# tpatten/squirrel_motion_planner

Hardware: AMD Instinct MI355X
Metric: collision-checked samples/sec + time-to-first-feasible-path, 8-DoF, 5 cm octomap (higher is better)
Workload: dtype f64

## Files before the change

squirrel_motion_planner_amd/csrc/smp_kernels.hip:

```cpp
#include <hip/hip_runtime.h>

#include <vector>

#include "smp_collide.h"
#include "smp_math.h"
#include "smp_plan.h"
#include "smp_types.h"

extern "C" __device__ __attribute__((const)) unsigned long long __ockl_wfred_min_u64(unsigned long long);
extern "C" __device__ __attribute__((const)) unsigned long long __ockl_wfred_max_u64(unsigned long long);

namespace smp {

constexpr int CHECK_CT = 32;

__shared__ RobotDev g_rb;
__shared__ MapCfg g_mc;
__shared__ WideStash g_wk;

__device__ __forceinline__ void stage_model(const RobotDev* rb, const MapCfg* mc, RobotDev* rbl, MapCfg* mcl) {
  static_assert(sizeof(RobotDev) % 8 == 0 && sizeof(MapCfg) % 4 == 0, "staging granularity");
  for (int i = threadIdx.x; i < (int)(sizeof(RobotDev) / 8); i += BLOCK)
    reinterpret_cast<uint64_t*>(rbl)[i] = reinterpret_cast<const uint64_t*>(rb)[i];
  for (int i = threadIdx.x; i < (int)(sizeof(MapCfg) / 4); i += BLOCK)
// ... 335 lines not shown
  NodeRef sel;
  double sel_start[NJ], sel_target[NJ];
  double csp[3], best_nv;
  double sol[3];
  double wd[BLOCK / 64];
  unsigned long long wk[BLOCK / 64];
  int wi[BLOCK / 64];
  long long wcount[BLOCK / 64];
  ScoutRec sr;
  PreRec prer;
  int prer_ok;
#ifdef SMP_TRACE
  int trole;
  unsigned tn;
  long long tit;
#endif
  int sp_on, sp_stage, sp_go[2];
  double fnn_d;
  int fnn_id;
#ifdef SMP_SCAN_PROF
  unsigned long long spc_t;
#endif
  int sc_same[MAX_SCOUTS];
  unsigned sc_seen, sc_dead;
  int asked[SCOUT_SLOTS];
  int asked_conn[SCOUT_SLOTS];
  int asked_pre[SCOUT_SLOTS];
  int conn_rec;
  int two_scouts;
  unsigned sc_mod;
  unsigned rw_at0;
  int n_at0;
  int sc_t, sc_rerun;
  int rb_go[2];
  long long sc_k;
  int eg_hit[MAXE];
  int eg_rec[MAXE];
  int rec_grp;
  int rec_all, ev_job;
  double pc_q[2][PATCH_K][NJ];
};

__shared__ PlanLds g_L;

struct Ctx {
  SceneDev sc;
  QueryDev Q;
};

#ifdef SMP_TRACE
#ifndef SMP_TRACE_IT0
#define SMP_TRACE_IT0 3000
#endif
#ifndef SMP_TRACE_IT1
#define SMP_TRACE_IT1 3040
#endif
constexpr unsigned TLOG_CAP = 1u << 18, TLOG_ROLE = TLOG_CAP / 4;
__device__ unsigned long long g_tlog[TLOG_CAP];
__device__ unsigned g_tlog_n[4];
#define TR()                                                                                                  \
  if (threadIdx.x == 0 && g_L.tit >= SMP_TRACE_IT0 && g_L.tit < SMP_TRACE_IT1 && g_L.tn < TLOG_ROLE) {        \
    g_tlog[g_L.trole * TLOG_ROLE + g_L.tn] =                                                                   \
        ((unsigned long long)g_L.trole << 62) | ((unsigned long long)((g_L.tit - SMP_TRACE_IT0) & 0xff) << 54) | \
        ((unsigned long long)(__LINE__ & 0x3fff) << 40) | (wall_clock64() & 0xffffffffffull);                  \
    g_tlog_n[g_L.trole] = ++g_L.tn;                                                                            \
  }
// ... 1687 lines not shown
      const int c = threadIdx.x / NJ, j = threadIdx.x - c * NJ;
      const int sl = base + c, k = sl / J.np1, i = sl - k * J.np1;
      J.tq[c][j] = J.start[k][j] + i * J.step[k][j];
    }
    if (threadIdx.x < TILE_CT_MAX) J.T.coll[threadIdx.x] = 0;
    __syncthreads();
  }
  const TileOrder order{J.tgrp, J.tord, J.first, false};
  collide_wide((&g_rb), K, ct, nc, J.tq, self, map, J.T, sk ? &order : nullptr, prof);
  unsigned m = 0;
  for (int c = 0; c < nc; ++c) m |= (J.T.coll[c] ? 1u : 0u) << c;
  if (sync_after) __syncthreads();
  return m;
}

__device__ __noinline__ unsigned job_tile_mask_out(const Ctx& C, JobLds& J, int t, int seq) {
  const WideConst K = wide_const_load(g_wk, C.sc);
  return job_tile_mask(C, K, J, t, nullptr, seq);
}

enum { OV_NONE = 0, OV_NEAR_EXPAND = 1, OV_NN = 2, OV_NEAR_XN = 3 };
__device__ void overlap_work(const Ctx& C, int ov, int t);
__device__ __forceinline__ bool take_spec(int ov) {
  const bool hit = uni(g_L.spec) == ov;
  __syncthreads();
  if (hit && threadIdx.x == 0) {
    (ov == OV_NN ? g_L.S.nn_nodes : g_L.S.near_nodes) += g_L.spec_cnt;
    g_L.spec = OV_NONE;
  }
  __syncthreads();
  return hit;
}

__device__ __forceinline__ void edge_validity_job(const Ctx& C, int E, int pslot, int ov, int ovt, bool sfv) {
  JobBoard* jb = C.Q.jb;
  auto& J = g_L.u.job;
  const int np1 = g_L.S.n_pts + 1;
  const int W = max(1, C.Q.nworkers);
  if (threadIdx.x < 64) {
    const int e = threadIdx.x;
    const bool need = e < E && g_L.eg_need[e] && g_L.eg_hit[e] < 0;
    const unsigned long long m = __ballot(need);
    const int k = __popcll(m & ((1ull << e) - 1));
    if (need) J.emap[k] = e;
    if (e == 0) {
      const int ne = __popcll(m);
      J.E = ne;
      J.np1 = np1;
      J.nslots = ne * np1;
      J.ct = job_tile_ct(ne * np1, W, C.Q.tile_ct);
      J.ntiles = (ne * np1 + J.ct - 1) / J.ct;
      J.self = g_L.S.self; J.map = g_L.S.map;
      J.seq = ++g_L.job_seq;
#ifdef SMP_NO_SKIP
      J.skip = 0;
#else
      J.skip = J.ntiles > W;
#endif
      J.sfv = J.skip && sfv;
    }
  }
  if (threadIdx.x < E) g_L.eg_first[threadIdx.x] = np1;
  __syncthreads();
  const int ne = uni(J.E), nt = uni(J.ntiles), seq = uni(J.seq), ct = uni(J.ct);
  if (ne == 0) {
    overlap_work(C, OV_NONE, ovt);
    return;
  }
  const unsigned long long tj0 = threadIdx.x == 0 ? wall_clock64() : 0;
  for (int it = threadIdx.x; it < ne * NJ; it += BLOCK) {
    const int k = it / NJ, j = it - k * NJ, e = J.emap[k];
    J.start[k][j] = g_L.eg_start[e][j];
    J.step[k][j] = g_L.eg_step[e][j];
  }
  for (int t = threadIdx.x; t < nt; t += BLOCK) J.rdone[t] = 0;
  if (threadIdx.x < ne) J.first[threadIdx.x] = np1;
  __syncthreads();
  for (int i = threadIdx.x; i < 1 + 32 * ne; i += BLOCK) {
    unsigned w;
    if (i == 0) {
      w = (unsigned)ne | (unsigned)np1 << 8 | (unsigned)(J.self != 0) << 16 | (unsigned)(J.map != 0) << 17 |
          (unsigned)J.skip << 19 | (unsigned)J.sfv << 20 | (unsigned)__builtin_ctz((unsigned)J.ct) << 21;
    } else {
      const int m = i - 1, k = m >> 5, r = m & 31, j = (r & 15) >> 1;
      const unsigned long long bits = (unsigned long long)__double_as_longlong(r < 16 ? J.start[k][j] : J.step[k][j]);
      w = (r & 1) ? (unsigned)(bits >> 32) : (unsigned)bits;
    }
    st_agent(&jb->pay[i], granule(seq, w));
  }
#ifdef SMP_JOB_PROF
  if (threadIdx.x == 0) st_agent(&jb->dbg[0], wall_clock64());
#endif
  PROF_BEGIN();
  if (threadIdx.x == 0) { g_L.S.prof[P_TFK] += _pt - tj0; g_L.S.prof[P_TTEST]++; }
  TR();
  if (threadIdx.x == 0) g_L.in_job = 1;
  __syncthreads();
  overlap_work(C, ov, ovt);
  if (threadIdx.x == 0) g_L.in_job = 0;
  TR();
  const bool skip = uni(J.skip) != 0;
  for (int t = W - 1; t < nt; t += W) {
    const unsigned m = job_tile_mask_out(C, J, t, skip ? seq : -1);
    if (threadIdx.x == 0) {
      J.rmask[t] = m;
      J.rdone[t] = 1;
      if (skip) st_agent(&jb->res[t], granule(seq, m));
    }
  }
  __syncthreads();
  const unsigned long long tj1 = threadIdx.x == 0 ? wall_clock64() : 0;
  if (threadIdx.x == 0) g_L.S.prof[P_TCHAIN] += tj1 - _pt;
  unsigned long long t_prog = tj1, t_wait = tj1;
  int last_left = 1 << 30;
  for (int k = 0;; k ^= 1) {
    if (threadIdx.x < 64) {
      int left = 0;
      for (int t = threadIdx.x; t < nt; t += 64) {
        if (J.rdone[t]) continue;
        const unsigned long long v = ld_agent(&jb->res[t]);
        if ((int)(v >> 32) == seq) { J.rmask[t] = (unsigned)v; J.rdone[t] = 1; }
        else ++left;
      }
      left = __ockl_wfred_add_i32(left);
      if (threadIdx.x == 0) {
        const unsigned long long now = wall_clock64();
        if (left != last_left) { last_left = left; t_prog = now; }
        int st = left == 0 ? 1 : (now - t_prog > 800ull ? 2 : 0);
        if (st != 1 && now - t_wait > 200000000ull) {
          g_L.S.status = -5;
          g_L.S.phase = 2;
          g_L.S.prof[28] = (unsigned long long)left;
          g_L.S.prof[29] = (unsigned long long)nt;
          g_L.S.prof[31] = (unsigned long long)seq;
          st = 1;
        }
        J.go[k] = st;
      }
    }
    __syncthreads();
    const int go = uni(J.go[k]);
    if (go == 1) break;
    if (go == 2) {
      if (threadIdx.x < 64) {
        int cand = 1 << 30;
        for (int t = threadIdx.x; t < nt; t += 64)
          if (!J.rdone[t]) { cand = t; break; }
        cand = __ockl_wfred_min_i32(cand);
        if (threadIdx.x == 0) J.steal = cand < nt ? cand : -1;
      }
      __syncthreads();
      const int t = uni(J.steal);
      if (t >= 0) {
        const unsigned m = job_tile_mask_out(C, J, t, -1);
        if (threadIdx.x == 0) { J.rmask[t] = m; J.rdone[t] = 1; }
      }
// ... 773 lines not shown
      }
    }
    if (e < MAXE) g_L.eg_rec[e] = m;
    const unsigned long long miss = __ballot(e < E && m < 0);
    if (e == 0) { g_L.rec_grp = sgrp; g_L.rec_all = miss == 0; }
  }
  __syncthreads();
  return uni(g_L.rec_all) != 0;
}

__device__ void edge_costs_rec(int E) {
  const int np = g_L.S.n_pts;
  if (threadIdx.x < E * NJ) {
    const int e = threadIdx.x / NJ, j = threadIdx.x - e * NJ;
    const double st = (g_L.eg_target[e][j] - g_L.eg_start[e][j]) / double(np);
    g_L.eg_step[e][j] = st;
    g_L.eg_end[e][j] = g_L.eg_start[e][j] + np * st;
  } else if (threadIdx.x >= 256 && threadIdx.x < 256 + E * 3) {
    const int i = threadIdx.x - 256, e = i / 3, k = i - e * 3;
    const double a = g_L.sr.e[g_L.eg_rec[e]].acc[k];
    g_L.eg_acc[e][k] = a;
    g_L.eg_cost[e][k] = g_L.eg_base[e][k] + a;
  }
  __syncthreads();
}

__device__ __noinline__ void local_tile(const Ctx& C, int nc) {
  const TileOrder order{g_L.tile_e, g_L.tile_i, g_L.eg_first, false};
  collide_tile<PLAN_CT>((&g_rb), C.sc, (&g_mc), nc, g_L.u.tile.tq, g_L.S.self, g_L.S.map, g_L.u.tile.T, &order,
                        &g_L.S.prof[P_TFK]);
}

__device__ __forceinline__ void edge_validity(const Ctx& C, int E, bool stop_first_valid, int pslot, int ov = 0, int ovt = 0,
                              int sgrp = -1) {
  const int np1 = g_L.S.n_pts + 1;
  if (threadIdx.x == 0) g_L.count_slot = pslot + 4;
  TR();
  if (C.Q.jb) {
    const bool matched = uni(g_L.rec_grp) == sgrp && sgrp >= 0;
    const bool rec = sgrp >= 0 && (matched || spec_stage(C, sgrp));
    TR();
    if (threadIdx.x < 64) {
      const int e = threadIdx.x;
      const bool need = e < E && g_L.eg_need[e];
      int hit = -2;
      if (rec && need) {
        if (matched) {
          const int k = g_L.eg_rec[e];
          if (k >= 0 && g_L.sr.e[k].first >= 0) hit = g_L.sr.e[k].first;
        } else {
          const int g0 = sgrp == SC_EXPAND ? 0 : sgrp == SC_CHOOSE ? SCOUT_CHOOSE0 : SCOUT_REWIRE0;
          const int gn = sgrp == SC_EXPAND ? 1 : sgrp == SC_CHOOSE ? g_L.sr.n_choose : g_L.sr.n_rewire;
          const int d = e < gn ? e : -1;
          for (int u = 0; u < gn; ++u) {
            const int k = g0 + (d < 0 ? u : (u == 0 ? d : (u <= d ? u - 1 : u)));
            const ScoutEdge& R = g_L.sr.e[k];
            if (R.first >= 0 && same8(g_L.eg_start[e], R.s) && same8(g_L.eg_target[e], R.g)) { hit = R.first; break; }
          }
        }
      }
      if (e < MAXE) g_L.eg_hit[e] = hit;
      const unsigned long long mh = __ballot(need && hit >= 0), mm = __ballot(need && hit < 0);
      if (rec && e == 0) { g_L.S.sc_edge_hit += __popcll(mh); g_L.S.sc_edge_miss += __popcll(mm); }
      if (mm == 0 && e < E) g_L.eg_first[e] = need ? hit : np1;
      if (e == 0) {
        g_L.ev_job = mm != 0;
        g_L.rec_grp = -1;
        if (mm == 0) g_L.spec = OV_NONE;
      }
    }
    __syncthreads();
    if (!uni(g_L.ev_job)) { TR(); return; }
    edge_validity_job(C, E, pslot, ov, ovt, stop_first_valid);
    if (threadIdx.x < E && g_L.eg_hit[threadIdx.x] >= 0) g_L.eg_first[threadIdx.x] = g_L.eg_hit[threadIdx.x];
    __syncthreads();
    TR();
    return;
  }
  if (threadIdx.x < E) { g_L.eg_first[threadIdx.x] = np1; g_L.eg_ptr[threadIdx.x] = 0; }
  __syncthreads();
  for (;;) {
    if (threadIdx.x < 64) {
      const int e = threadIdx.x;
      const bool live = e < E && g_L.eg_need[e] && g_L.eg_first[e] >= np1;
      const int ptr = e < E ? g_L.eg_ptr[e] : np1;
      bool stop = false;
      if (stop_first_valid) {
        const unsigned long long m = __ballot(live);
        if (m) stop = __shfl(ptr, __builtin_ctzll(m)) >= np1;
      }
      const int rem = (live && ptr < np1) ? np1 - ptr : 0;
      int inc = rem;
      for (int off = 1; off < 32; off <<= 1) {
        int v = __shfl_up(inc, off);
        if (e >= off) inc += v;
      }
      const int start = inc - rem;
      const int take = stop ? 0 : max(0, min(rem, PLAN_CT - start));
      for (int i = 0; i < take; ++i) { g_L.tile_e[start + i] = e; g_L.tile_i[start + i] = ptr + i; }
      if (e < E) g_L.eg_ptr[e] = ptr + take;
      const int total = __shfl(inc, 31);
      if (e == 0) g_L.tile_n = stop ? 0 : min(PLAN_CT, total);
    }
    __syncthreads();
    const int nc = uni(g_L.tile_n);
    if (nc == 0) break;
    if (threadIdx.x < nc * NJ) {
      int c = threadIdx.x / NJ, j = threadIdx.x - c * NJ;
      int e = g_L.tile_e[c];
      g_L.u.tile.tq[c][j] = g_L.eg_start[e][j] + g_L.tile_i[c] * g_L.eg_step[e][j];
    }
    __syncthreads();
// ... 709 lines not shown
    __syncthreads();
    if (C.Q.jb && rec_match(C, E, SC_CHOOSE)) edge_costs_rec(E);
    else edge_costs(C, E);
    if (threadIdx.x < E) g_L.eg_need[threadIdx.x] = g_L.eg_cost[threadIdx.x][0] <= g_L.xn.c[0];
    for (int e = E + threadIdx.x; e < MAXE; e += BLOCK) g_L.eg_need[e] = 0;
    __syncthreads();
    edge_validity(C, E, true, P_XCHOOSE, 0, 0, SC_CHOOSE);
    count_edges(E, true);
    if (threadIdx.x == 0) {
      if (g_L.found >= 0) {
        g_L.ext_bp = 1;
        g_L.n_via = 0;
        g_L.nn_t = g_L.S.n[t];
        load_node(C, t, g_L.eg_near[g_L.found], &g_L.cur);
      }
    }
    __syncthreads();
    if (uni(g_L.found) >= 0) {
      via_chain(C, g_L.xn.q);
      if (threadIdx.x == 0) {
        g_L.xn.id = g_L.sel.id;
        g_L.xn.parent = g_L.sel.parent;
        for (int j = 0; j < NJ; ++j) g_L.xn.q[j] = g_L.sel.q[j];
        for (int k = 0; k < 3; ++k) g_L.xn.c[k] = g_L.sel.c[k];
        for (int j = 0; j < NJ; ++j) { g_L.en_start[j] = g_L.sel_start[j]; g_L.en_target[j] = g_L.sel_target[j]; }
      }
      __syncthreads();
      insert_via(C, t);
    }
  }
  __syncthreads();
}

__device__ void rewire_count(const TreeDev& T) {
  if (threadIdx.x < 64) {
    const int n = g_L.nk, lane = threadIdx.x;
    const int m = n >= g_L.S.max_near ? g_L.S.max_near : n;
    bool ok = false;
    if (lane < m) {
      int hv = g_L.n_hi - 1 - lane;
      BCHK(hv, MAX_NEAR, __LINE__, 9);
      int v = g_L.hi_i[hv];
      BCHK(v, g_L.S.cap, __LINE__, 9);
      ok = g_L.xn.c[0] < T.cost[v];
    }
    const int cnt = __popcll(__ballot(ok));
    if (lane == 0) g_L.cnt = cnt;
  }
  __syncthreads();
}

__device__ void rewire(const Ctx& C, int t) {
  const int cap = g_L.S.cap;
  const TreeDev& T = C.Q.tr[t];
  rewire_count(T);
  const int cnt = uni(g_L.cnt);
  if (cnt == 0) return;
  if (threadIdx.x < cnt) {
    int e = threadIdx.x;
    int pos = g_L.n_hi - 1 - e;
    int v = g_L.hi_i[pos];
    NodeRef nd;
    load_node(C, t, v, &nd);
    for (int j = 0; j < NJ; ++j) { g_L.eg_start[e][j] = g_L.xn.q[j]; g_L.eg_target[e][j] = nd.q[j]; }
    for (int k = 0; k < 3; ++k) g_L.eg_base[e][k] = g_L.xn.c[k];
    g_L.eg_near[e] = v;
  }
// ... 964 lines not shown
  if (threadIdx.x == 0) {
    S.n[t] = Xn;
    S.n[1 - t] = XBn;
    S.prof[26]++;
    R.cn.ok = 0;
    R.pre.ok = 0;
    R.nn.ok = 0; R.ex.ok = 0; R.nr.ok = 0; R.n_choose = 0; R.n_rewire = 0; R.cc.ok = 0; R.cc.nfirst = -1;
  }
  __syncthreads();
  return true;
}

__device__ void scout_iteration(const Ctx& C, long long it, int t, int X, int opt, unsigned ver, int XB) {
  QState& S = g_L.S;
  ScoutRec& R = g_L.sr;
  ScoutBoard* sb = C.Q.scb;
  JobBoard* jb = C.Q.jb;
  const int par = (int)(it & (SCOUT_SLOTS - 1));
  const unsigned tag = (unsigned)(it + 1);
  (void)jb;
  unsigned long long _ts = threadIdx.x == 0 ? pclk() : 0;
#ifdef SMP_TRACE
  if (threadIdx.x == 0) g_L.tit = it;
#endif
  TR();
  if (threadIdx.x == 0) {
    S.prof[30]++;
    S.n[t] = X;
    S.n[1 - t] = XB;
    R.cn.ok = 0;
    R.pre.ok = 0;
    R.nn.ok = 0; R.ex.ok = 0; R.nr.ok = 0; R.n_choose = 0; R.n_rewire = 0; R.cc.ok = 0; R.cc.nfirst = -1;
  }
  if (opt) sc_publish(C, par, tag, SC_STARTED);
  if (threadIdx.x < 64) {
    const JobBoard* lb = C.Q.sampler_jb;
    const unsigned want = ring_tag(it, ver);
    const unsigned long long t0 = wall_clock64();
    int ok = 0;
    for (;;) {
      unsigned long long v = 0;
      if (threadIdx.x < 2 * NJ) v = ld_agent(&lb->ring[it % SMP_RING].g[threadIdx.x]);
      const bool cur = threadIdx.x >= 2 * NJ || (unsigned)(v >> 32) == want;
      if (__ballot(!cur) == 0) {
        const unsigned hi = (unsigned)odd_lane_of_pair((int)(unsigned)v);
        if (threadIdx.x < 2 * NJ && !(threadIdx.x & 1))
          g_L.xr[threadIdx.x >> 1] = __longlong_as_double((long long)(((unsigned long long)hi << 32) | (unsigned)v));
        ok = 1;
        break;
      }
      if (__builtin_amdgcn_readfirstlane((int)(wall_clock64() - t0 > 2000))) break;
      __builtin_amdgcn_s_sleep(2);
    }
    if (threadIdx.x == 0) g_L.flag = ok;
  }
  __syncthreads();
  SC_PHASE(0);
  TR();
  if (!uni(g_L.flag) && !opt) {
    scout_pre_publish(C, par, tag, false);
    return;
  }
  if (!uni(g_L.flag)) {
    sc_copy_out(sb, par, &R.nn, sizeof(ScoutNN));
    sc_copy_out(sb, par, &R.nr, sizeof(ScoutNear));
    sc_copy_out(sb, par, &R.cn, sizeof(ScoutConnect));
    sc_copy_out(sb, par, &R.pre, sizeof(ScoutPre));
    sc_copy_out(sb, par, &R.n_choose, 4 * sizeof(int));
    sc_end(C, par, tag, opt);
    return;
  }
  int rp = 0;
redo:
  if (opt && sc_moved(C)) return;
  int nid;
// ... 7 lines not shown
    for (int j = 0; j < NJ; ++j) { nq[j] = g_L.nn.q[j]; xe[j] = g_L.xr[j]; }
    double s = 0.0;
#pragma unroll
    for (int j = 0; j < NJ; ++j) { const double d = xe[j] - nq[j]; s += d * d; }
    const double d = sqrt(s);
    const double nn_l = g_L.nn.q[lane & 7];
    double x_l = g_L.xr[lane & 7];
    step_towards_w(rev_mask(&g_rb), nq, xe, S.step, lane, nn_l, x_l);
    if (lane < NJ) {
      R.nn.q[lane] = g_L.xr[lane];
      g_L.ext[lane] = x_l;
      g_L.eg_start[0][lane] = nn_l;
      g_L.eg_target[0][lane] = x_l;
    } else if (lane < NJ + 3) {
      const int k = lane - NJ;
      R.nn.c[k] = g_L.nn.c[k];
      g_L.eg_base[0][k] = g_L.nn.c[k];
    } else if (lane == NJ + 3) {
      R.nn.d = d < 10000.0 ? d : 10000.0;
      R.nn.id = nid; R.nn.X = X; R.nn.t = t; R.nn.ok = 1;
      g_L.eg_need[0] = 1;
    }
  }
  __syncthreads();
  if (opt) {
    sc_copy_out(sb, par, &R.nn, sizeof(ScoutNN));
    sc_publish(C, par, tag, SC_NN);
  }
  SC_PHASE(1);
  TR();
  if (opt && sc_moved(C)) return;
  edge_costs(C, 1);
  if (threadIdx.x == 0) {
    for (int j = 0; j < NJ; ++j) { R.ex.ext[j] = g_L.eg_target[0][j]; R.ex.step[j] = g_L.eg_step[0][j]; R.ex.end[j] = g_L.eg_end[0][j]; }
    for (int k = 0; k < 3; ++k) R.ex.acc[k] = g_L.eg_acc[0][k];
    R.ex.ok = 1;
  }
  if (threadIdx.x == 0) g_L.spec = OV_NONE;
  const bool spec_conn = !opt && !sc_stale(C, tag);
  int cid_s = 0;
  if (spec_conn) {
    const int tb = 1 - t;
    [[clang::always_inline]] cid_s = nearest(C, tb, g_L.eg_end[0]);
    if (threadIdx.x == 0) {
      load_node(C, tb, cid_s, &g_L.xc);
      for (int j = 0; j < NJ; ++j) { g_L.eg_start[1][j] = g_L.xc.q[j]; g_L.eg_target[1][j] = g_L.eg_end[0][j]; }
      for (int k = 0; k < 3; ++k) g_L.eg_base[1][k] = g_L.xc.c[k];
      g_L.eg_need[1] = 1;
    }
    for (int e = 2 + threadIdx.x; e < MAXE; e += BLOCK) g_L.eg_need[e] = 0;
    __syncthreads();
    edge_costs(C, 2);
    [[clang::always_inline]] edge_validity(C, 2, false, P_XEXPAND, OV_NONE, t);
  } else {
    [[clang::always_inline]] edge_validity(C, 1, false, P_XEXPAND, opt ? OV_NEAR_EXPAND : OV_NONE, t);
  }
  if (threadIdx.x == 0) {
    for (int j = 0; j < NJ; ++j) { R.e[0].s[j] = g_L.eg_start[0][j]; R.e[0].g[j] = g_L.eg_target[0][j]; }
    for (int k = 0; k < 3; ++k) R.e[0].acc[k] = g_L.eg_acc[0][k];
    R.e[0].first = g_L.eg_first[0];
    const int f = g_L.eg_first[0];
    g_L.ext_nn = f > S.n_pts;
    if (g_L.ext_nn) {
      for (int j = 0; j < NJ; ++j) g_L.xn.q[j] = g_L.eg_end[0][j];
      for (int k = 0; k < 3; ++k) g_L.xn.c[k] = g_L.eg_cost[0][k];
    } else {
      for (int j = 0; j < NJ; ++j) g_L.xn.q[j] = g_L.xr[j];
      g_L.xn.c[0] = 10000.0; g_L.xn.c[1] = 0.0; g_L.xn.c[2] = 0.0;
    }
    g_L.xn.id = X;
    g_L.xn.parent = g_L.nn.id;
    g_L.ext_bp = 0;
  }
  __syncthreads();
  if (!opt && (C.Q.pre_refresh & 1) && rp < 2 && pre_newer(C, t, X, XB)) {
    X = uni(g_L.cnt);
    XB = uni(g_L.found);
    rp++;
    goto redo;
  }
  if (opt) {
    sc_copy_out(sb, par, &R.e[0], sizeof(ScoutEdge));
    sc_copy_out(sb, par, &R.ex, sizeof(ScoutExpand));
  }
  if (spec_conn && uni(g_L.ext_nn)) {
    const int tb = 1 - t;
    const int cid = cid_s;
    if (threadIdx.x < NJ) {
      const int j = threadIdx.x;
      g_L.eg_start[0][j] = g_L.eg_start[1][j]; g_L.eg_target[0][j] = g_L.eg_target[1][j];
      g_L.eg_step[0][j] = g_L.eg_step[1][j]; g_L.eg_end[0][j] = g_L.eg_end[1][j];
    }
    if (threadIdx.x < 3) {
      const int k = threadIdx.x;
      g_L.eg_base[0][k] = g_L.eg_base[1][k]; g_L.eg_acc[0][k] = g_L.eg_acc[1][k]; g_L.eg_cost[0][k] = g_L.eg_cost[1][k];
    }
    if (threadIdx.x == 0) {
      g_L.eg_first[0] = g_L.eg_first[1];
      double s = 0.0;
      for (int j = 0; j < NJ; ++j) { double d = g_L.xn.q[j] - g_L.xc.q[j]; s += d * d; }
      const double d = sqrt(s);
      for (int j = 0; j < NJ; ++j) R.cn.q[j] = g_L.xn.q[j];
      R.cn.d = d < 10000.0 ? d : 10000.0;
      R.cn.id = cid; R.cn.X = XB; R.cn.t = tb;
    }
    __syncthreads();
    if (threadIdx.x == 0) {
      for (int j = 0; j < NJ; ++j) { R.cn.e.s[j] = g_L.eg_start[0][j]; R.cn.e.g[j] = g_L.eg_target[0][j]; }
      for (int k = 0; k < 3; ++k) { R.cn.e.acc[k] = g_L.eg_acc[0][k]; R.cn.c[k] = g_L.xc.c[k]; }
      R.cn.e.first = g_L.eg_first[0];
      R.cn.ok = 1;
    }
    __syncthreads();
    scout_pre_connect(C, par, tb);
  }
  if (!opt && (C.Q.pre_refresh & 2) && rp < 2 && pre_newer(C, t, X, XB)) {
    X = uni(g_L.cnt);
    XB = uni(g_L.found);
    rp++;
    goto redo;
  }
  if (!opt) {
    scout_pre_publish(C, par, tag, true);
    return;
  }
  if (sc_stale(C, tag)) {
    sc_copy_out(sb, par, &R.nr, sizeof(ScoutNear));
    sc_copy_out(sb, par, &R.n_choose, 4 * sizeof(int));
    sc_publish(C, par, tag, SC_DONE);
    return;
  }
  sc_publish(C, par, tag, SC_EXPAND);
  SC_PHASE(2);
  TR();
  if (sc_moved(C)) return;
  if (!(uni(g_L.ext_nn) && take_spec(OV_NEAR_EXPAND))) {
    [[clang::always_inline]] near_set<20>(C, t, g_L.xn.q, X);
  }
  if (threadIdx.x < 20) {
    R.nr.lo_i[threadIdx.x] = g_L.lo_i[threadIdx.x]; R.nr.lo_c[threadIdx.x] = g_L.lo_c[threadIdx.x];
    R.nr.hi_i[threadIdx.x] = g_L.hi_i[threadIdx.x]; R.nr.hi_c[threadIdx.x] = g_L.hi_c[threadIdx.x];
  }
  if (threadIdx.x == 0) {
    for (int j = 0; j < NJ; ++j) R.nr.q[j] = g_L.xn.q[j];
    R.nr.nk = g_L.nk; R.nr.n_lo = g_L.n_lo; R.nr.n_hi = g_L.n_hi;
    R.nr.X = X; R.nr.t = t; R.nr.ok = 1;
  }
  __syncthreads();
  sc_copy_out(sb, par, &R.nr, sizeof(ScoutNear));
  sc_publish(C, par, tag, SC_NEAR);
  SC_PHASE(3);
  TR();
  if (sc_moved(C)) return;
  if (threadIdx.x < 64) {
    const int E = choose_prefix();
    if (threadIdx.x == 0) {
      g_L.cnt = E;
      g_L.found = -1;
    }
  }
  __syncthreads();
  const int E = uni(g_L.cnt);
  if (E > 0) {
    if (threadIdx.x < E) {
      const int e = threadIdx.x;
      NodeRef nd;
      load_node(C, t, g_L.lo_i[e], &nd);
      for (int j = 0; j < NJ; ++j) { g_L.eg_start[e][j] = nd.q[j]; g_L.eg_target[e][j] = g_L.xn.q[j]; }
      for (int k = 0; k < 3; ++k) g_L.eg_base[e][k] = nd.c[k];
      g_L.eg_near[e] = nd.id;
    }
    __syncthreads();
    edge_costs(C, E);
    if (threadIdx.x < E) g_L.eg_need[threadIdx.x] = g_L.eg_cost[threadIdx.x][0] <= g_L.xn.c[0];
    for (int e = E + threadIdx.x; e < MAXE; e += BLOCK) g_L.eg_need[e] = 0;
    __syncthreads();
    [[clang::always_inline]] edge_validity(C, E, false, P_XCHOOSE);
    if (threadIdx.x < E) {
      const int e = threadIdx.x;
      ScoutEdge& w = R.e[SCOUT_CHOOSE0 + e];
      for (int j = 0; j < NJ; ++j) { w.s[j] = g_L.eg_start[e][j]; w.g[j] = g_L.eg_target[e][j]; }
      for (int k = 0; k < 3; ++k) w.acc[k] = g_L.eg_acc[e][k];
      w.first = g_L.eg_need[e] ? g_L.eg_first[e] : -1;
    }
    if (threadIdx.x < 64) {
      const bool fr = (int)threadIdx.x < E && g_L.eg_need[threadIdx.x] && g_L.eg_first[threadIdx.x] > S.n_pts;
      const unsigned long long fm = __ballot(fr);
      if (threadIdx.x == 0) {
        R.n_choose = E;
        if (fm) g_L.found = (int)__builtin_ctzll(fm);
      }
    }
    __syncthreads();
  }
  sc_copy_out(sb, par, &R.n_choose, 4 * sizeof(int));
  sc_copy_out(sb, par, &R.e[SCOUT_CHOOSE0], E * (int)sizeof(ScoutEdge));
  if (sc_stale(C, tag)) { sc_publish(C, par, tag, SC_DONE); return; }
  sc_publish(C, par, tag, SC_CHOOSE);
  SC_PHASE(4);
  TR();
  if (uni(g_L.found) >= 0) {
    if (threadIdx.x == 0) {
      g_L.n_via = 0;
      g_L.nn_t = X;
      load_node(C, t, g_L.eg_near[g_L.found], &g_L.cur);
    }
    __syncthreads();
    via_chain(C, g_L.xn.q);
    if (threadIdx.x == 0) {
      g_L.xn.id = g_L.sel.id;
      g_L.xn.parent = g_L.sel.parent;
      for (int j = 0; j < NJ; ++j) g_L.xn.q[j] = g_L.sel.q[j];
      for (int k = 0; k < 3; ++k) g_L.xn.c[k] = g_L.sel.c[k];
      g_L.ext_bp = 1;
      g_L.n_via = 0;
    }
    __syncthreads();
  }
  SC_PHASE(5);
  TR();
  if (!uni(g_L.ext_nn || g_L.ext_bp)) { sc_end(C, par, tag, opt); return; }
  if (sc_moved(C)) return;
  const TreeDev& T = C.Q.tr[t];
  rewire_count(T);
  const int cnt = uni(g_L.cnt);
  if (cnt > 0) {
    if (threadIdx.x < cnt) {
      const int e = threadIdx.x, v = g_L.hi_i[g_L.n_hi - 1 - e];
      NodeRef nd;
      load_node(C, t, v, &nd);
      for (int j = 0; j < NJ; ++j) { g_L.eg_start[e][j] = g_L.xn.q[j]; g_L.eg_target[e][j] = nd.q[j]; }
      for (int k = 0; k < 3; ++k) g_L.eg_base[e][k] = g_L.xn.c[k];
      g_L.eg_near[e] = v;
    }
    __syncthreads();
    edge_costs(C, cnt);
    if (threadIdx.x < cnt) {
      const int e = threadIdx.x, v = g_L.eg_near[e];
      g_L.eg_need[e] = (v != g_L.xn.parent) && (T.parent[v] != 0) && (g_L.eg_cost[e][0] < T.cost[v]);
    }
    for (int e = cnt + threadIdx.x; e < MAXE; e += BLOCK) g_L.eg_need[e] = 0;
    __syncthreads();
    [[clang::always_inline]] edge_validity(C, cnt, false, P_XREWIRE);
    if (threadIdx.x < cnt) {
      const int e = threadIdx.x;
      ScoutEdge& w = R.e[SCOUT_REWIRE0 + e];
      for (int j = 0; j < NJ; ++j) { w.s[j] = g_L.eg_start[e][j]; w.g[j] = g_L.eg_target[e][j]; }
      for (int k = 0; k < 3; ++k) w.acc[k] = g_L.eg_acc[e][k];
      w.first = g_L.eg_need[e] ? g_L.eg_first[e] : -1;
    }
    if (threadIdx.x == 0) R.n_rewire = cnt;
    __syncthreads();
  }
  sc_copy_out(sb, par, &R.n_choose, 4 * sizeof(int));
  sc_copy_out(sb, par, &R.e[SCOUT_REWIRE0], cnt * (int)sizeof(ScoutEdge));
  sc_publish(C, par, tag, SC_DONE);
  SC_PHASE(6);
  TR();
  if (sc_moved(C)) return;
  if (uni(g_L.two_scouts)) {
    [[clang::always_inline]] scout_connect(C, it, t, par, tag);
  }
  TR();
}
#undef SC_PHASE

__device__ __forceinline__ void scout_ctx(Ctx& C, int which) {
  C.Q.scb = C.Q.scbs[which];
  C.Q.sjb = C.Q.sjbs[which];
  C.Q.svia = C.Q.svias[which];
  C.Q.sworkers = C.Q.sworkers_s[which];
  C.Q.sampler_jb = C.Q.jb;
  C.Q.jb = C.Q.sjb;
  C.Q.nworkers = C.Q.sworkers;
  C.Q.via = C.Q.svia;
  C.Q.rows = nullptr;
  C.Q.trace = nullptr;
  C.Q.ttff = nullptr;
}

__device__ __noinline__ void scout_main(Ctx& C, int which) {
  {
    const int* src = reinterpret_cast<const int*>(C.Q.st);
    int* dst = reinterpret_cast<int*>(&g_L.S);
    for (int i = threadIdx.x; i < (int)(sizeof(QState) / sizeof(int)); i += BLOCK) dst[i] = src[i];
  }
  __syncthreads();
  if (threadIdx.x < 32) g_L.S.prof[threadIdx.x] = 0;
// ... 586 lines not shown
```

squirrel_motion_planner_amd/csrc/smp_plan.h:

```cpp
#pragma once
#include <stdint.h>

#include "smp_types.h"

namespace smp {

constexpr int MAX_PTS = 32;
constexpr int MAX_NEAR = 32;
#ifndef SMP_MAXE
#define SMP_MAXE 24
#endif
constexpr int MAXE = SMP_MAXE;

struct NodeRef {
  double q[NJ];
  double c[3];
  int id;
  int parent;
};

struct TreeDev {
  double* q;
  double* cost;
  int* parent;
  int* first_child;
  int* next_sib;
  int* prev_sib;
  double* e_start;
  double* e_target;
  float* qf;
};

struct QState {
// ... 71 lines not shown
  unsigned long long res[JOB_TILES];
  int pad2[32 - (2 * JOB_TILES) % 32];
  unsigned long long spay[64];
  int s_ver, s_have_sol;
  long long s_iter;
  unsigned long long s_cbest[3];
  int pad6[22];
  struct {
    unsigned long long g[RING_G];
  } ring[SMP_RING];
  unsigned long long sres[SCAN_P][SCAN_W];
};

constexpr int SCOUT_EDGES = 1 + 2 * MAX_NEAR;
constexpr int SCOUT_CHOOSE0 = 1, SCOUT_REWIRE0 = 1 + MAX_NEAR;
enum { SC_STARTED = 0, SC_NN = 1, SC_EXPAND = 2, SC_NEAR = 3, SC_CHOOSE = 4, SC_DONE = 5, SC_CONN = 6 };
struct ScoutNN {
  double q[NJ];
  double d;
  double c[3];
  int id, X, t, ok;
};
struct ScoutNear {
  double q[NJ];
  int nk, n_lo, n_hi, ok, X, t;
  int lo_i[MAX_NEAR], hi_i[MAX_NEAR];
  double lo_c[MAX_NEAR], hi_c[MAX_NEAR];
};
struct ScoutEdge {
  double s[NJ], g[NJ];
  double acc[3];
  int first, pad;
};
struct ScoutExpand {
  double ext[NJ];
  double step[NJ], end[NJ];
  double acc[3];
  int ok, pad;
};
struct ScoutConnect {
  double q[NJ];
  double d;
  double c[3];
  int id, X, t, ok;
  ScoutEdge e;
};
constexpr int PRE_VIA = 16;
struct ScoutPre {
  int ok;
  int flag;
  int nv, need;
  double sol[3];
  NodeRef sel;
  double sel_start[NJ], sel_target[NJ];
};
struct ScoutConn {
  double q[NJ];
  double d;
  int id, X, t, excl;
  int nk, n_lo, n_hi, ok;
  int lo_i[MAX_NEAR], hi_i[MAX_NEAR];
  double lo_c[MAX_NEAR], hi_c[MAX_NEAR];
  double acc0[3];
  double pad0;
  double acc[MAX_NEAR][3];
  int first0, nfirst;
// ... 94 lines not shown
```

Baseline: 4.527 million.

## Publish scout edge records early and overlap staleness checks with job wait

Scout edge and expand records are now written to the shared scout board while the collision job is in flight, rather than copied out after validity checking. Only the per-edge 'first' field is sent afterward. The job header is built inside the hit-check pass, the payload is written before the local copy, and the staleness flag is read during the result-polling loop. Near-node data for rewire is prefetched during the near phase, and the sampler ring is loaded before publishing. This removes serial global-memory copy-outs and extra syncs from the scout's critical path, at the cost of more shared state and subtle ordering that scout consumers depend on.

Result: faster. 4.640 million, median of 6 (+2.5%).

```diff
diff --git a/squirrel_motion_planner_amd/csrc/smp_kernels.hip b/squirrel_motion_planner_amd/csrc/smp_kernels.hip
--- a/squirrel_motion_planner_amd/csrc/smp_kernels.hip
+++ b/squirrel_motion_planner_amd/csrc/smp_kernels.hip
@@ -391,6 +391,9 @@
   unsigned rw_at0;
   int n_at0;
   int sc_t, sc_rerun;
+  int sc_stale_f;
+  double sc_hq[MAXE][NJ], sc_hc[MAXE];
+  int sc_hp[MAXE];
   int rb_go[2];
   long long sc_k;
   int eg_hit[MAXE];
@@ -2144,62 +2147,102 @@
   return hit;
 }
 
-__device__ __forceinline__ void edge_validity_job(const Ctx& C, int E, int pslot, int ov, int ovt, bool sfv) {
+enum { EARLY_NONE = 0, EARLY_EXPAND = 1, EARLY_CHOOSE = 2, EARLY_REWIRE = 3 };
+constexpr int EDGE_EARLY_W = (int)(offsetof(ScoutEdge, first) / 8);
+static_assert(EDGE_EARLY_W == 2 * NJ + 3, "ScoutEdge: s, g, acc, then {first, pad}");
+__device__ __forceinline__ int sc_stale_now(const ScoutBoard* sb) {
+  return (long long)ld_agent(&sb->cur) > g_L.sc_k || ld_agent(&sb->stop);
+}
+__device__ __forceinline__ void sc_early_send(const Ctx& C, int early, int epar, int E, bool read_stale) {
+  if (early == EARLY_NONE) return;
+  ScoutBoard* sb = C.Q.scb;
+  ScoutRec* rec = &sb->rec[epar];
+  if (read_stale && threadIdx.x == 0) g_L.sc_stale_f = sc_stale_now(sb);
+  const int g0 = early == EARLY_EXPAND ? 0 : early == EARLY_CHOOSE ? SCOUT_CHOOSE0 : SCOUT_REWIRE0;
+  for (int i = threadIdx.x; i < E * EDGE_EARLY_W; i += BLOCK) {
+    const int e = i / EDGE_EARLY_W, k = i - e * EDGE_EARLY_W;
+    const double v = k < NJ ? g_L.eg_start[e][k] : k < 2 * NJ ? g_L.eg_target[e][k - NJ] : g_L.eg_acc[e][k - 2 * NJ];
+    st_agent(reinterpret_cast<unsigned long long*>(&rec->e[g0 + e]) + k, (unsigned long long)__double_as_longlong(v));
+  }
+  if (early == EARLY_EXPAND) {
+    constexpr int XW = (int)(sizeof(ScoutExpand) / 8);
+    static_assert(XW == 3 * NJ + 3 + 1 && offsetof(ScoutExpand, ok) == (XW - 1) * 8, "ScoutExpand: ext, step, end, acc, {ok, pad}");
+    const int k = (int)threadIdx.x - 64;
+    if (k >= 0 && k < XW) {
+      unsigned long long w;
+      if (k == XW - 1) w = *reinterpret_cast<const unsigned long long*>(&g_L.sr.ex.ok);
+      else w = (unsigned long long)__double_as_longlong(k < NJ ? g_L.eg_target[0][k] : k < 2 * NJ ? g_L.eg_step[0][k - NJ] :
+                                                        k < 3 * NJ ? g_L.eg_end[0][k - 2 * NJ] : g_L.eg_acc[0][k - 3 * NJ]);
+      st_agent(reinterpret_cast<unsigned long long*>(&rec->ex) + k, w);
+    }
+  } else {
+    const int k = (int)threadIdx.x - (BLOCK - 64);
+    if (k >= 0 && k < 2) st_agent(reinterpret_cast<unsigned long long*>(&rec->n_choose) + k,
+                                  reinterpret_cast<const unsigned long long*>(&g_L.sr.n_choose)[k]);
+  }
+}
+__device__ __forceinline__ void sc_first_send(const Ctx& C, int early, int epar, int E) {
+  const int g0 = early == EARLY_EXPAND ? 0 : early == EARLY_CHOOSE ? SCOUT_CHOOSE0 : SCOUT_REWIRE0;
+  if ((int)threadIdx.x < E) {
+    const int e = threadIdx.x;
+    const int first = g_L.eg_need[e] ? g_L.eg_first[e] : -1;
+    st_agent(reinterpret_cast<unsigned long long*>(&C.Q.scb->rec[epar].e[g0 + e]) + EDGE_EARLY_W,
+             (unsigned long long)(unsigned)first);
+  }
+}
+
+__device__ __forceinline__ void job_header(const Ctx& C, bool need, bool sfv) {
+  auto& J = g_L.u.job;
+  const int e = threadIdx.x;
+  const int np1 = g_L.S.n_pts + 1;
+  const int W = max(1, C.Q.nworkers);
+  const unsigned long long m = __ballot(need);
+  const int k = __popcll(m & ((1ull << e) - 1));
+  if (need) J.emap[k] = e;
+  if (e == 0) {
+    const int ne = __popcll(m);
+    J.E = ne;
+    J.np1 = np1;
+    J.nslots = ne * np1;
+    J.ct = job_tile_ct(ne * np1, W, C.Q.tile_ct);
+    J.ntiles = (ne * np1 + J.ct - 1) / J.ct;
+    J.self = g_L.S.self; J.map = g_L.S.map;
+    J.seq = ++g_L.job_seq;
+#ifdef SMP_NO_SKIP
+    J.skip = 0;
+#else
+    J.skip = J.ntiles > W;
+#endif
+    J.sfv = J.skip && sfv;
+  }
+}
+__device__ __forceinline__ void edge_validity_job(const Ctx& C, int E, int pslot, int ov, int ovt, int early = 0,
+                                                  int epar = 0) {
   JobBoard* jb = C.Q.jb;
   auto& J = g_L.u.job;
   const int np1 = g_L.S.n_pts + 1;
   const int W = max(1, C.Q.nworkers);
-  if (threadIdx.x < 64) {
-    const int e = threadIdx.x;
-    const bool need = e < E && g_L.eg_need[e] && g_L.eg_hit[e] < 0;
-    const unsigned long long m = __ballot(need);
-    const int k = __popcll(m & ((1ull << e) - 1));
-    if (need) J.emap[k] = e;
-    if (e == 0) {
-      const int ne = __popcll(m);
-      J.E = ne;
-      J.np1 = np1;
-      J.nslots = ne * np1;
-      J.ct = job_tile_ct(ne * np1, W, C.Q.tile_ct);
-      J.ntiles = (ne * np1 + J.ct - 1) / J.ct;
-      J.self = g_L.S.self; J.map = g_L.S.map;
-      J.seq = ++g_L.job_seq;
-#ifdef SMP_NO_SKIP
-      J.skip = 0;
-#else
-      J.skip = J.ntiles > W;
-#endif
-      J.sfv = J.skip && sfv;
-    }
-  }
-  if (threadIdx.x < E) g_L.eg_first[threadIdx.x] = np1;
-  __syncthreads();
   const int ne = uni(J.E), nt = uni(J.ntiles), seq = uni(J.seq), ct = uni(J.ct);
-  if (ne == 0) {
-    overlap_work(C, OV_NONE, ovt);
-    return;
-  }
   const unsigned long long tj0 = threadIdx.x == 0 ? wall_clock64() : 0;
-  for (int it = threadIdx.x; it < ne * NJ; it += BLOCK) {
-    const int k = it / NJ, j = it - k * NJ, e = J.emap[k];
-    J.start[k][j] = g_L.eg_start[e][j];
-    J.step[k][j] = g_L.eg_step[e][j];
-  }
-  for (int t = threadIdx.x; t < nt; t += BLOCK) J.rdone[t] = 0;
-  if (threadIdx.x < ne) J.first[threadIdx.x] = np1;
-  __syncthreads();
   for (int i = threadIdx.x; i < 1 + 32 * ne; i += BLOCK) {
     unsigned w;
     if (i == 0) {
       w = (unsigned)ne | (unsigned)np1 << 8 | (unsigned)(J.self != 0) << 16 | (unsigned)(J.map != 0) << 17 |
           (unsigned)J.skip << 19 | (unsigned)J.sfv << 20 | (unsigned)__builtin_ctz((unsigned)J.ct) << 21;
     } else {
-      const int m = i - 1, k = m >> 5, r = m & 31, j = (r & 15) >> 1;
-      const unsigned long long bits = (unsigned long long)__double_as_longlong(r < 16 ? J.start[k][j] : J.step[k][j]);
+      const int m = i - 1, k = m >> 5, r = m & 31, j = (r & 15) >> 1, e = J.emap[k];
+      const unsigned long long bits = (unsigned long long)__double_as_longlong(r < 16 ? g_L.eg_start[e][j] : g_L.eg_step[e][j]);
       w = (r & 1) ? (unsigned)(bits >> 32) : (unsigned)bits;
     }
     st_agent(&jb->pay[i], granule(seq, w));
   }
+  for (int it = threadIdx.x; it < ne * NJ; it += BLOCK) {
+    const int k = it / NJ, j = it - k * NJ, e = J.emap[k];
+    J.start[k][j] = g_L.eg_start[e][j];
+    J.step[k][j] = g_L.eg_step[e][j];
+  }
+  for (int t = threadIdx.x; t < nt; t += BLOCK) J.rdone[t] = 0;
+  if (threadIdx.x < ne) J.first[threadIdx.x] = np1;
 #ifdef SMP_JOB_PROF
   if (threadIdx.x == 0) st_agent(&jb->dbg[0], wall_clock64());
 #endif
@@ -2207,6 +2250,7 @@
   if (threadIdx.x == 0) { g_L.S.prof[P_TFK] += _pt - tj0; g_L.S.prof[P_TTEST]++; }
   TR();
   if (threadIdx.x == 0) g_L.in_job = 1;
+  sc_early_send(C, early, epar, E, false);
   __syncthreads();
   overlap_work(C, ov, ovt);
   if (threadIdx.x == 0) g_L.in_job = 0;
@@ -2228,12 +2272,16 @@
   for (int k = 0;; k ^= 1) {
     if (threadIdx.x < 64) {
       int left = 0;
+      unsigned long long cur_v = 0;
+      int stop_v = 0;
+      if (early != EARLY_NONE && threadIdx.x == 0) { cur_v = ld_agent(&C.Q.scb->cur); stop_v = ld_agent(&C.Q.scb->stop); }
       for (int t = threadIdx.x; t < nt; t += 64) {
         if (J.rdone[t]) continue;
         const unsigned long long v = ld_agent(&jb->res[t]);
         if ((int)(v >> 32) == seq) { J.rmask[t] = (unsigned)v; J.rdone[t] = 1; }
         else ++left;
       }
+      if (early != EARLY_NONE && threadIdx.x == 0) g_L.sc_stale_f = (long long)cur_v > g_L.sc_k || stop_v;
       left = __ockl_wfred_add_i32(left);
       if (threadIdx.x == 0) {
         const unsigned long long now = wall_clock64();
@@ -3073,7 +3121,7 @@
 }
 
 __device__ __forceinline__ void edge_validity(const Ctx& C, int E, bool stop_first_valid, int pslot, int ov = 0, int ovt = 0,
-                              int sgrp = -1) {
+                              int sgrp = -1, int early = 0, int epar = 0) {
   const int np1 = g_L.S.n_pts + 1;
   if (threadIdx.x == 0) g_L.count_slot = pslot + 4;
   TR();
@@ -3103,7 +3151,8 @@
       if (e < MAXE) g_L.eg_hit[e] = hit;
       const unsigned long long mh = __ballot(need && hit >= 0), mm = __ballot(need && hit < 0);
       if (rec && e == 0) { g_L.S.sc_edge_hit += __popcll(mh); g_L.S.sc_edge_miss += __popcll(mm); }
-      if (mm == 0 && e < E) g_L.eg_first[e] = need ? hit : np1;
+      if (e < E) g_L.eg_first[e] = mm == 0 && need ? hit : np1;
+      if (mm != 0) job_header(C, need && hit < 0, stop_first_valid);
       if (e == 0) {
         g_L.ev_job = mm != 0;
         g_L.rec_grp = -1;
@@ -3111,14 +3160,24 @@
       }
     }
     __syncthreads();
-    if (!uni(g_L.ev_job)) { TR(); return; }
-    edge_validity_job(C, E, pslot, ov, ovt, stop_first_valid);
-    if (threadIdx.x < E && g_L.eg_hit[threadIdx.x] >= 0) g_L.eg_first[threadIdx.x] = g_L.eg_hit[threadIdx.x];
-    __syncthreads();
+    if (!uni(g_L.ev_job)) {
+      if (early != EARLY_NONE) {
+        sc_early_send(C, early, epar, E, true);
+        __syncthreads();
+      }
+      TR();
+      return;
+    }
+    edge_validity_job(C, E, pslot, ov, ovt, early, epar);
+    if (sgrp >= 0) {
+      if (threadIdx.x < E && g_L.eg_hit[threadIdx.x] >= 0) g_L.eg_first[threadIdx.x] = g_L.eg_hit[threadIdx.x];
+      __syncthreads();
+    }
     TR();
     return;
   }
   if (threadIdx.x < E) { g_L.eg_first[threadIdx.x] = np1; g_L.eg_ptr[threadIdx.x] = 0; }
+  sc_early_send(C, early, epar, E, true);
   __syncthreads();
   for (;;) {
     if (threadIdx.x < 64) {
@@ -3894,7 +3953,7 @@
   __syncthreads();
 }
 
-__device__ void rewire_count(const TreeDev& T) {
+__device__ __noinline__ void rewire_count(const TreeDev& T) {
   if (threadIdx.x < 64) {
     const int n = g_L.nk, lane = threadIdx.x;
     const int m = n >= g_L.S.max_near ? g_L.S.max_near : n;
@@ -4925,15 +4984,17 @@
     R.pre.ok = 0;
     R.nn.ok = 0; R.ex.ok = 0; R.nr.ok = 0; R.n_choose = 0; R.n_rewire = 0; R.cc.ok = 0; R.cc.nfirst = -1;
   }
+  unsigned long long v0 = 0;
+  if (threadIdx.x < 2 * NJ) v0 = ld_agent(&C.Q.sampler_jb->ring[it % SMP_RING].g[threadIdx.x]);
   if (opt) sc_publish(C, par, tag, SC_STARTED);
   if (threadIdx.x < 64) {
     const JobBoard* lb = C.Q.sampler_jb;
     const unsigned want = ring_tag(it, ver);
     const unsigned long long t0 = wall_clock64();
     int ok = 0;
-    for (;;) {
-      unsigned long long v = 0;
-      if (threadIdx.x < 2 * NJ) v = ld_agent(&lb->ring[it % SMP_RING].g[threadIdx.x]);
+    for (bool first_round = true;; first_round = false) {
+      unsigned long long v = v0;
+      if (!first_round && threadIdx.x < 2 * NJ) v = ld_agent(&lb->ring[it % SMP_RING].g[threadIdx.x]);
       const bool cur = threadIdx.x >= 2 * NJ || (unsigned)(v >> 32) == want;
       if (__ballot(!cur) == 0) {
         const unsigned hi = (unsigned)odd_lane_of_pair((int)(unsigned)v);
@@ -5007,8 +5068,10 @@
   if (opt && sc_moved(C)) return;
   edge_costs(C, 1);
   if (threadIdx.x == 0) {
-    for (int j = 0; j < NJ; ++j) { R.ex.ext[j] = g_L.eg_target[0][j]; R.ex.step[j] = g_L.eg_step[0][j]; R.ex.end[j] = g_L.eg_end[0][j]; }
-    for (int k = 0; k < 3; ++k) R.ex.acc[k] = g_L.eg_acc[0][k];
+    if (!opt) {
+      for (int j = 0; j < NJ; ++j) { R.ex.ext[j] = g_L.eg_target[0][j]; R.ex.step[j] = g_L.eg_step[0][j]; R.ex.end[j] = g_L.eg_end[0][j]; }
+      for (int k = 0; k < 3; ++k) R.ex.acc[k] = g_L.eg_acc[0][k];
+    }
     R.ex.ok = 1;
   }
   if (threadIdx.x == 0) g_L.spec = OV_NONE;
@@ -5028,12 +5091,16 @@
     edge_costs(C, 2);
     [[clang::always_inline]] edge_validity(C, 2, false, P_XEXPAND, OV_NONE, t);
   } else {
-    [[clang::always_inline]] edge_validity(C, 1, false, P_XEXPAND, opt ? OV_NEAR_EXPAND : OV_NONE, t);
-  }
+    [[clang::always_inline]] edge_validity(C, 1, false, P_XEXPAND, opt ? OV_NEAR_EXPAND : OV_NONE, t, -1,
+                                           opt ? EARLY_EXPAND : EARLY_NONE, par);
+  }
+  if (opt) sc_first_send(C, EARLY_EXPAND, par, 1);
   if (threadIdx.x == 0) {
-    for (int j = 0; j < NJ; ++j) { R.e[0].s[j] = g_L.eg_start[0][j]; R.e[0].g[j] = g_L.eg_target[0][j]; }
-    for (int k = 0; k < 3; ++k) R.e[0].acc[k] = g_L.eg_acc[0][k];
-    R.e[0].first = g_L.eg_first[0];
+    if (!opt) {
+      for (int j = 0; j < NJ; ++j) { R.e[0].s[j] = g_L.eg_start[0][j]; R.e[0].g[j] = g_L.eg_target[0][j]; }
+      for (int k = 0; k < 3; ++k) R.e[0].acc[k] = g_L.eg_acc[0][k];
+      R.e[0].first = g_L.eg_first[0];
+    }
     const int f = g_L.eg_first[0];
     g_L.ext_nn = f > S.n_pts;
     if (g_L.ext_nn) {
@@ -5054,10 +5121,6 @@
     rp++;
     goto redo;
   }
-  if (opt) {
-    sc_copy_out(sb, par, &R.e[0], sizeof(ScoutEdge));
-    sc_copy_out(sb, par, &R.ex, sizeof(ScoutExpand));
-  }
   if (spec_conn && uni(g_L.ext_nn)) {
     const int tb = 1 - t;
     const int cid = cid_s;
@@ -5099,7 +5162,7 @@
     scout_pre_publish(C, par, tag, true);
     return;
   }
-  if (sc_stale(C, tag)) {
+  if (uni(g_L.sc_stale_f)) {
     sc_copy_out(sb, par, &R.nr, sizeof(ScoutNear));
     sc_copy_out(sb, par, &R.n_choose, 4 * sizeof(int));
     sc_publish(C, par, tag, SC_DONE);
@@ -5121,56 +5184,57 @@
     R.nr.nk = g_L.nk; R.nr.n_lo = g_L.n_lo; R.nr.n_hi = g_L.n_hi;
     R.nr.X = X; R.nr.t = t; R.nr.ok = 1;
   }
-  __syncthreads();
-  sc_copy_out(sb, par, &R.nr, sizeof(ScoutNear));
-  sc_publish(C, par, tag, SC_NEAR);
-  SC_PHASE(3);
-  TR();
-  if (sc_moved(C)) return;
   if (threadIdx.x < 64) {
     const int E = choose_prefix();
     if (threadIdx.x == 0) {
       g_L.cnt = E;
       g_L.found = -1;
-    }
-  }
-  __syncthreads();
+      R.n_choose = E;
+    }
+  }
+  __syncthreads();
+  sc_copy_out(sb, par, &R.nr, sizeof(ScoutNear));
   const int E = uni(g_L.cnt);
+  if (threadIdx.x < E) {
+    const int e = threadIdx.x;
+    NodeRef nd;
+    load_node(C, t, g_L.lo_i[e], &nd);
+    for (int j = 0; j < NJ; ++j) { g_L.eg_start[e][j] = nd.q[j]; g_L.eg_target[e][j] = g_L.xn.q[j]; }
+    for (int k = 0; k < 3; ++k) g_L.eg_base[e][k] = nd.c[k];
+    g_L.eg_near[e] = nd.id;
+  } else if (threadIdx.x >= 64 && (int)threadIdx.x - 64 < min(g_L.n_hi, MAXE)) {
+    const TreeDev& T = C.Q.tr[t];
+    const int i = (int)threadIdx.x - 64, v = g_L.hi_i[i], cap = g_L.S.cap;
+    BCHK(v, cap, __LINE__, t);
+    double q[NJ];
+    for (int j = 0; j < NJ; ++j) q[j] = T.q[(size_t)j * cap + v];
+    const double c0 = T.cost[v];
+    const int pv = T.parent[v];
+    for (int j = 0; j < NJ; ++j) g_L.sc_hq[i][j] = q[j];
+    g_L.sc_hc[i] = c0;
+    g_L.sc_hp[i] = pv;
+  }
+  sc_publish(C, par, tag, SC_NEAR);
+  SC_PHASE(3);
+  TR();
+  if (sc_moved(C)) return;
   if (E > 0) {
-    if (threadIdx.x < E) {
-      const int e = threadIdx.x;
-      NodeRef nd;
-      load_node(C, t, g_L.lo_i[e], &nd);
-      for (int j = 0; j < NJ; ++j) { g_L.eg_start[e][j] = nd.q[j]; g_L.eg_target[e][j] = g_L.xn.q[j]; }
-      for (int k = 0; k < 3; ++k) g_L.eg_base[e][k] = nd.c[k];
-      g_L.eg_near[e] = nd.id;
-    }
-    __syncthreads();
     edge_costs(C, E);
     if (threadIdx.x < E) g_L.eg_need[threadIdx.x] = g_L.eg_cost[threadIdx.x][0] <= g_L.xn.c[0];
     for (int e = E + threadIdx.x; e < MAXE; e += BLOCK) g_L.eg_need[e] = 0;
     __syncthreads();
-    [[clang::always_inline]] edge_validity(C, E, false, P_XCHOOSE);
-    if (threadIdx.x < E) {
-      const int e = threadIdx.x;
-      ScoutEdge& w = R.e[SCOUT_CHOOSE0 + e];
-      for (int j = 0; j < NJ; ++j) { w.s[j] = g_L.eg_start[e][j]; w.g[j] = g_L.eg_target[e][j]; }
-      for (int k = 0; k < 3; ++k) w.acc[k] = g_L.eg_acc[e][k];
-      w.first = g_L.eg_need[e] ? g_L.eg_first[e] : -1;
-    }
+    [[clang::always_inline]] edge_validity(C, E, false, P_XCHOOSE, OV_NONE, 0, -1, EARLY_CHOOSE, par);
+    sc_first_send(C, EARLY_CHOOSE, par, E);
     if (threadIdx.x < 64) {
       const bool fr = (int)threadIdx.x < E && g_L.eg_need[threadIdx.x] && g_L.eg_first[threadIdx.x] > S.n_pts;
       const unsigned long long fm = __ballot(fr);
-      if (threadIdx.x == 0) {
-        R.n_choose = E;
-        if (fm) g_L.found = (int)__builtin_ctzll(fm);
-      }
-    }
-    __syncthreads();
-  }
-  sc_copy_out(sb, par, &R.n_choose, 4 * sizeof(int));
-  sc_copy_out(sb, par, &R.e[SCOUT_CHOOSE0], E * (int)sizeof(ScoutEdge));
-  if (sc_stale(C, tag)) { sc_publish(C, par, tag, SC_DONE); return; }
+      if (threadIdx.x == 0 && fm) g_L.found = (int)__builtin_ctzll(fm);
+    }
+    if (uni(g_L.sc_stale_f)) { sc_publish(C, par, tag, SC_DONE); return; }
+  } else {
+    sc_copy_out(sb, par, &R.n_choose, 4 * sizeof(int));
+    if (sc_stale(C, tag)) { sc_publish(C, par, tag, SC_DONE); return; }
+  }
   sc_publish(C, par, tag, SC_CHOOSE);
   SC_PHASE(4);
   TR();
@@ -5196,39 +5260,39 @@
   TR();
   if (!uni(g_L.ext_nn || g_L.ext_bp)) { sc_end(C, par, tag, opt); return; }
   if (sc_moved(C)) return;
-  const TreeDev& T = C.Q.tr[t];
-  rewire_count(T);
+  if (threadIdx.x < 64) {
+    const int n = g_L.nk, lane = threadIdx.x;
+    const int m = min(n >= S.max_near ? S.max_near : n, min(g_L.n_hi, MAXE));
+    const bool ok = lane < m && g_L.xn.c[0] < g_L.sc_hc[g_L.n_hi - 1 - lane];
+    const int c = __popcll(__ballot(ok));
+    if (lane == 0) g_L.cnt = c;
+  }
+  __syncthreads();
   const int cnt = uni(g_L.cnt);
   if (cnt > 0) {
-    if (threadIdx.x < cnt) {
-      const int e = threadIdx.x, v = g_L.hi_i[g_L.n_hi - 1 - e];
-      NodeRef nd;
-      load_node(C, t, v, &nd);
-      for (int j = 0; j < NJ; ++j) { g_L.eg_start[e][j] = g_L.xn.q[j]; g_L.eg_target[e][j] = nd.q[j]; }
+    if (threadIdx.x < cnt * NJ) {
+      const int e = threadIdx.x / NJ, j = threadIdx.x - e * NJ;
+      g_L.eg_start[e][j] = g_L.xn.q[j];
+      g_L.eg_target[e][j] = g_L.sc_hq[g_L.n_hi - 1 - e][j];
+    } else if (threadIdx.x >= 256 && threadIdx.x < 256 + cnt) {
+      const int e = threadIdx.x - 256;
       for (int k = 0; k < 3; ++k) g_L.eg_base[e][k] = g_L.xn.c[k];
-      g_L.eg_near[e] = v;
+      g_L.eg_near[e] = g_L.hi_i[g_L.n_hi - 1 - e];
     }
     __syncthreads();
     edge_costs(C, cnt);
     if (threadIdx.x < cnt) {
-      const int e = threadIdx.x, v = g_L.eg_near[e];
-      g_L.eg_need[e] = (v != g_L.xn.parent) && (T.parent[v] != 0) && (g_L.eg_cost[e][0] < T.cost[v]);
+      const int e = threadIdx.x, v = g_L.eg_near[e], h = g_L.n_hi - 1 - e;
+      g_L.eg_need[e] = (v != g_L.xn.parent) && (g_L.sc_hp[h] != 0) && (g_L.eg_cost[e][0] < g_L.sc_hc[h]);
     }
     for (int e = cnt + threadIdx.x; e < MAXE; e += BLOCK) g_L.eg_need[e] = 0;
-    __syncthreads();
-    [[clang::always_inline]] edge_validity(C, cnt, false, P_XREWIRE);
-    if (threadIdx.x < cnt) {
-      const int e = threadIdx.x;
-      ScoutEdge& w = R.e[SCOUT_REWIRE0 + e];
-      for (int j = 0; j < NJ; ++j) { w.s[j] = g_L.eg_start[e][j]; w.g[j] = g_L.eg_target[e][j]; }
-      for (int k = 0; k < 3; ++k) w.acc[k] = g_L.eg_acc[e][k];
-      w.first = g_L.eg_need[e] ? g_L.eg_first[e] : -1;
-    }
     if (threadIdx.x == 0) R.n_rewire = cnt;
     __syncthreads();
-  }
-  sc_copy_out(sb, par, &R.n_choose, 4 * sizeof(int));
-  sc_copy_out(sb, par, &R.e[SCOUT_REWIRE0], cnt * (int)sizeof(ScoutEdge));
+    [[clang::always_inline]] edge_validity(C, cnt, false, P_XREWIRE, OV_NONE, 0, -1, EARLY_REWIRE, par);
+    sc_first_send(C, EARLY_REWIRE, par, cnt);
+  } else {
+    sc_copy_out(sb, par, &R.n_choose, 4 * sizeof(int));
+  }
   sc_publish(C, par, tag, SC_DONE);
   SC_PHASE(6);
   TR();
diff --git a/squirrel_motion_planner_amd/csrc/smp_plan.h b/squirrel_motion_planner_amd/csrc/smp_plan.h
--- a/squirrel_motion_planner_amd/csrc/smp_plan.h
+++ b/squirrel_motion_planner_amd/csrc/smp_plan.h
@@ -1,4 +1,5 @@
 #pragma once
+#include <stddef.h>
 #include <stdint.h>
 
 #include "smp_types.h"
@@ -136,6 +137,8 @@
   double acc[3];
   int first, pad;
 };
+static_assert(offsetof(ScoutEdge, first) % 8 == 0 && sizeof(ScoutEdge) - offsetof(ScoutEdge, first) == 8,
+              "ScoutEdge: {first, pad} is the last 8-byte word");
 struct ScoutExpand {
   double ext[NJ];
   double step[NJ], end[NJ];
```
